# themeshpotato/rust-ray-tracing-in-a-weekend

Hardware: AMD Instinct MI355X
Metric: Msamples/s (pixels x spp) for 1200x800 random-spheres scene (higher is better)
Workload: dtype f64

## Files before the change

rust-ray-tracing-in-a-weekend_amd/csrc/abi.cpp:

```cpp
#include <hip/hip_runtime.h>

#include <algorithm>
#include <array>
#include <limits>
#include <cmath>
#include <cstdio>
#include <cstdlib>
#include <cstring>
#include <new>
#include <string>
#include <vector>

#include "rt/rt_abi.h"
#include "adaptive_criterion.hpp"
#include "ctx_internal.hpp"
#include "deal_cache.hpp"
#include "denoise.hpp"
#include "features_kernel.hpp"
#include "launch_plan.hpp"
#include "scene_lower.hpp"
#include "scene_model.hpp"
#include "trace_kernel.hpp"

namespace {
// ... 487 lines not shown
        const void* src;
        size_t bytes, off;
    } t[10] = {{L.nodes.data(), L.nodes.size() * sizeof(rt_bvh_node), 0},
               {s->prim_refs, (size_t)s->n_prim_refs * 4, 0},
               {L.prims.data(), L.prims.size() * sizeof(rt_prim), 0},
               {L.instances.data(), L.instances.size() * sizeof(rt_instance), 0},
               {s->materials, (size_t)s->n_materials * sizeof(rt_material), 0},
               {s->textures, (size_t)s->n_textures * sizeof(rt_texture), 0},
               {s->perlin_ranvec, (size_t)s->n_perlin * 768 * 8, 0},
               {s->perlin_perm, (size_t)s->n_perlin * 768 * 4, 0},
               {s->image_data, (size_t)s->image_bytes, 0},
               {L.leaf_prims.data(), L.leaf_prims.size() * sizeof(rt_prim), 0}};
    size_t total = 0;
    for (Table& e : t) {
        e.off = total;
        total = align_up(total + e.bytes, 256);
    }
    total = std::max<size_t>(total, 256);
    HIP_TRY(hipSetDevice(c->device));
    HIP_TRY(hipStreamSynchronize(c->stream));
    if (c->any_enqueued) HIP_TRY(hipEventSynchronize(c->ev_done));
    if (total > c->scene_bytes) {
        (void)hipFree(c->scene_buf);
        c->scene_buf = nullptr;
        c->scene_bytes = 0;
        HIP_TRY(hipMalloc(&c->scene_buf, total));
        c->scene_bytes = total;
    }
    char* base = (char*)c->scene_buf;
    for (const Table& e : t)
        if (e.bytes) HIP_TRY(hipMemcpy(base + e.off, e.src, e.bytes, hipMemcpyHostToDevice));

    rtk::SceneDev& S = c->S;
    S.nodes = (const rt_bvh_node*)(base + t[0].off);
    S.prim_refs = (const int32_t*)(base + t[1].off);
    S.prims = (const rt_prim*)(base + t[2].off);
    S.instances = (const rt_instance*)(base + t[3].off);
    S.materials = (const rt_material*)(base + t[4].off);
    S.textures = (const rt_texture*)(base + t[5].off);
    S.perlin_ranvec = (const double*)(base + t[6].off);
    S.perlin_perm = (const int32_t*)(base + t[7].off);
    S.image = (const uint8_t*)(base + t[8].off);
    S.leaf_prims = (const rt_prim*)(base + t[9].off);
    S.tlas_root = s->tlas_root;
    S.pre_leaf = L.pre_leaf;
    S.pre_root = L.pre_root;
    std::copy(L.pre_lo, L.pre_lo + 3, S.pre_lo);
    std::copy(L.pre_hi, L.pre_hi + 3, S.pre_hi);
    S.stack16_ok = L.stack16_ok;
    S.blas_base = L.blas_base;
    S.stack_entries = L.stack_entries;
    S.n_tlas_nodes = L.n_tlas_nodes;
    S.n_blas_bfs = L.n_blas_bfs;
    S.n_lds_nodes = S.n_lds_blas = 0;
    S.has_lights = L.has_lights;
    S.has_spheres = L.has_spheres;
    c->scene = rtp::scene_facts(L, *s);
    c->has_scene = true;
    c->stats.scene_bytes = (int64_t)total;
    return RT_OK;
}

int rt_ctx_upload_world(rt_ctx* c, rt_world* w, int accel)
{
    const rt_scene_soa* soa = nullptr;
    int rc = rt_world_flatten(w, accel, &soa);
    if (rc) return rc;
    return rt_ctx_upload_soa(c, soa);
}

int rt_rows_in_shard(int height, int row_begin, int row_stride) { return rtp::rows_in_shard(height, row_begin, row_stride); }
int rt_rows_in_band_shard(int height, int row_begin, int row_stride, int row_block)
{
    return rtp::rows_in_band_shard(height, row_begin, row_stride, row_block);
}
int rt_tiles_in_shard(int width, int height, int tile_begin, int tile_stride)
{
    return rtp::tiles_in_shard(width, height, tile_begin, tile_stride);
}
using rtp::auto_chunk;
using rtp::bad_geometry;
using rtp::Layout;
using rtp::layout_of;
using rtp::row_block_of;

static int grow(rt_ctx* c, hipStream_t stream, double*& buf, size_t& cap, size_t need, bool* oom = nullptr)
{
    if (need <= cap) return RT_OK;
    HIP_TRY(hipStreamSynchronize(stream));
    (void)hipFree(buf);
    buf = nullptr;
    cap = 0;
    const hipError_t e = hipMalloc((void**)&buf, need);
    if (e == hipErrorOutOfMemory && oom) {
        (void)hipGetLastError();
        buf = nullptr;
        *oom = true;
        return RT_ERR_HIP;
    }
    HIP_TRY(e);
    cap = need;
    return RT_OK;
}

struct Sink {
    double* acc = nullptr;
    void* out = nullptr;
// ... 139 lines not shown
static int run_range(rt_ctx* c, const rt_camera* cam, const rt_render_params* p, int s_begin, int s_end, int chunk,
                     hipStream_t stream, const Sink& sink)
{
    const Layout lay = layout_of(p);
    const long long n_px = (long long)lay.rows * lay.w;
    if (n_px == 0 || s_end <= s_begin) {
        for (int i = 0; i < 3; ++i) HIP_TRY(hipEventRecord(c->ev[i], stream));
        write_stats(c, rtp::Plan{}, chunk, 0, false);
        c->last_deal_n = 0;
        return RT_OK;
    }

    const int64_t img_tiles = (int64_t)((p->width + 7) / 8) * ((p->height + 7) / 8);
    rtk::KParams K;
    int rc = fill_kparams(c, cam, p, lay, chunk, sink, img_tiles, K);
    if (rc) return rc;

    rtp::Request rq;
    rq.lay = lay;
    rq.s_begin = s_begin;
    rq.s_end = s_end;
    rq.chunk = chunk;
    rq.count_work = p->count_work != 0;
    rq.acc_sink = sink.acc != nullptr;
    rq.moments = sink.moments != nullptr;
    rq.cam_mag = rtp::camera_magnitude(*cam);
    rtp::Retry retry{c->sample_buf_cap, true};
    rtp::Plan pl;
    for (;;) {
        pl = rtp::plan(c->scene, c->dev, c->opt, rq, retry);
        if (pl.err) return fail(pl.err, pl.err_msg);
        rc = grow(c, stream, c->acc_tmp, c->acc_tmp_cap, pl.acc_bytes);
        if (rc) return rc;
        bool oom = false;
        rc = grow(c, stream, c->partial, c->partial_cap, pl.partial_bytes, &oom);
        if (rc == RT_OK && pl.ring) {
            rc = grow(c, stream, c->ring, c->ring_cap, pl.ring_bytes, &oom);
            if (rc != RT_OK && oom) {
                retry.ring_allowed = false;
                continue;
            }
        }
        if (rc == RT_OK) break;
        if (!oom) return rc;
        if (!rtp::shrink(pl, retry)) return hip_fail(hipErrorOutOfMemory, "trace output buffer (smallest batch)");
    }
    double* const open = pl.open_chunk ? c->acc_tmp : nullptr;
    double* const acc = !pl.own_total ? sink.acc : pl.open_chunk ? c->acc_tmp + pl.px * 3 : c->acc_tmp;
    rtk::SceneDev S = c->S;
    S.n_lds_nodes = pl.n_lds_nodes;
    S.n_lds_materials = pl.n_lds_materials;
    S.n_lds_textures = pl.n_lds_textures;
    S.n_lds_blas = pl.n_lds_blas;
    K.block_chunks = pl.block_chunks;
    K.block_samples = pl.block_samples;
    K.ring_waves = pl.ring_waves;
    int waves_per_simd = 0;
    rtk::LaunchOpts o;
    o.features = pl.features;
    o.slab32 = pl.slab32;
    o.lds_stack = pl.lds_stack;
    o.count = rq.count_work;
    o.pool = pl.schedule;
    o.f32 = pl.f32;
    o.waves_per_simd = &waves_per_simd;
    const rtk::SampleTiles tiles{lay.w, lay.rows, (lay.w + 7) / 8, pl.f32};
    rc = deal_setup(c, cam, p, pl, sink.moments != nullptr, img_tiles, stream, K);
    if (rc) return rc;

    if (pl.own_total) HIP_TRY(hipMemsetAsync(acc, 0, pl.px_bytes, stream));
    if (rq.count_work) {
        HIP_TRY(hipMemsetAsync(c->counters, 0, kCounters * sizeof(unsigned long long), stream));
        if (img_tiles > c->tile_cost_cap) {
            HIP_TRY(hipStreamSynchronize(stream));
            (void)hipFree(c->tile_cost);
            c->tile_cost = nullptr;
            c->tile_cost_cap = 0;
            HIP_TRY(hipMalloc((void**)&c->tile_cost, (size_t)img_tiles * sizeof(unsigned long long)));
            c->tile_cost_cap = img_tiles;
        }
        HIP_TRY(hipMemsetAsync(c->tile_cost, 0, (size_t)img_tiles * sizeof(unsigned long long), stream));
        K.tile_cost = c->tile_cost;
        c->tile_cost_n = pl.schedule == RT_SCHED_POOL || pl.schedule == RT_SCHED_ITEMS ? img_tiles : 0;
    }
    HIP_TRY(hipEventRecord(c->ev[0], stream));
    if (pl.overlap) {
        HIP_TRY(hipEventRecord(c->ev_in, stream));
        for (int i = 0; i < 2; ++i) HIP_TRY(hipStreamWaitEvent(c->tstream[i], c->ev_in, 0));
    }
    for (int bi = 0; bi < pl.n_batches; ++bi) {
        const int b0 = s_begin + (int)(bi * pl.batch);
        const int b1 = (int)std::min<long long>(s_end, b0 + pl.batch);
        K.sample_begin = b0;
        K.spp = b1;
        K.n_chunks = (b1 - b0 + chunk - 1) / chunk;
        {
            const bool items = pl.schedule == RT_SCHED_ITEMS;
            const unsigned g = items ? (unsigned)K.block_chunks : (unsigned)K.block_samples;
            const unsigned n = items ? (unsigned)K.n_chunks : (unsigned)(K.spp - K.sample_begin);
            const unsigned n_groups = (n + g - 1) / std::max(g, 1u);
            K.n_work_blocks = (unsigned)K.tiles_x * (unsigned)K.tiles_y * n_groups;
            K.deal_div = K.tile_major ? n_groups : (unsigned)K.tiles_x * (unsigned)K.tiles_y;
        }
        const int h = pl.overlap ? (bi & 1) : 0;
        double* buf = c->partial + (size_t)h * (pl.half_bytes / sizeof(double));
        hipStream_t ts = pl.overlap ? c->tstream[h] : stream;
// ... 932 lines not shown
```

rust-ray-tracing-in-a-weekend_amd/csrc/launch_plan.cpp:

```cpp
#include "launch_plan.hpp"

#include <algorithm>
#include <cmath>

#include "launch_shapes.hpp"
#include "scene_features.hpp"

namespace rtp {

namespace {

constexpr int kMaxLdsStack = 48;
constexpr int kMaxLdsNodes = 512;
#ifndef RT_MIN_WAVES_FINAL
#define RT_MIN_WAVES_FINAL 4
#endif
#ifndef RT_LDS_BLAS_MAX
#define RT_LDS_BLAS_MAX 1024
#endif
constexpr int kMaxLdsBlas = RT_LDS_BLAS_MAX;
constexpr int kMaxLdsMaterials = 64;

}

// ... 95 lines not shown
    const size_t px_bytes = pl.px_bytes = pl.px * 3 * sizeof(double);
    const size_t sample_bytes = pl.sample_bytes =
        rtk::tiled_pixels(rq.lay.w, n_rows) * 3 * (pl.f32 ? sizeof(float) : sizeof(double));
    pl.n_lds_nodes = opt.lds_nodes ? std::min(scene.n_tlas_nodes, kMaxLdsNodes) : 0;
    const bool stage = opt.lds_nodes && scene.n_materials <= kMaxLdsMaterials && scene.n_textures <= kMaxLdsMaterials &&
                       scene.n_materials > 0;
    pl.n_lds_materials = stage ? scene.n_materials : 0;
    pl.n_lds_textures = stage ? scene.n_textures : 0;
    pl.n_lds_blas = 0;
    if (scene.n_blas_bfs > 0 && opt.lds_nodes && (variant & rtk::FEAT_INST_BLAS) != 0) {
        const bool oct = pl.slab32 && pl.n_lds_nodes == scene.n_tlas_nodes && pl.n_lds_nodes > 0;
        const int bt = rtk::block_threads_of(variant, pl.f32 != 0);
        const size_t base = (size_t)pl.n_lds_nodes * (oct ? 80 : 64) +
                            (pl.lds_stack ? (size_t)scene.stack_entries * (size_t)bt * 4 : 0) +
                            (size_t)pl.n_lds_materials * 64 + (size_t)pl.n_lds_textures * 96;
        const size_t lds_cu = dev.lds_per_cu, granule = 1024;
        const size_t wave_blocks = std::max<size_t>(1, (size_t)(variant == rtk::FEAT_SET_FINAL ? 4 * RT_MIN_WAVES_FINAL : 12) /
                                                           (size_t)(bt / 64));
        const size_t blocks = std::max<size_t>(1, std::min(wave_blocks,
            lds_cu / (((std::max<size_t>(base, 1) + granule - 1) / granule) * granule)));
        const size_t budget = std::min(lds_cu / blocks, dev.lds_per_block) / granule * granule;
        const size_t spare = budget > base ? budget - base : 0;
        pl.n_lds_blas = (int32_t)std::min<size_t>({(size_t)scene.n_blas_bfs, spare / 64, (size_t)kMaxLdsBlas});
    }
    pl.block_chunks = opt.block_chunks > 0 ? opt.block_chunks : 2;
    if (opt.block_samples > 0) {
        pl.block_samples = opt.block_samples;
    } else {
        const long long tiles = (long long)((rq.lay.w + 7) / 8) * ((n_rows + 7) / 8);
        int bs = chunk;
        while (bs > 4 && tiles * ((total + bs - 1) / bs) < 160000) bs = (bs + 1) / 2;
        pl.block_samples = bs;
    }
    const bool ring_ok = retry.ring_allowed && opt.ring && pl.block_samples == chunk &&
                         chunk <= (int)(rtk::kRingSlot / 64) && rq.s_end <= (int)rtk::kRingSampleMask;
    const int ring_waves = dev.n_cus * (variant == rtk::FEAT_SET_SPHERES ? 24 : 20);
    const size_t ring_bytes = (size_t)ring_waves * rtk::kRingWaveDoubles * sizeof(double);
    const size_t buf_cap = retry.buf_cap;

    const bool cornell = variant == rtk::FEAT_SET_RECTINST;
    const bool fits_one = (size_t)total * sample_bytes <= buf_cap;
    pl.schedule = rq.moments                     ? RT_SCHED_POOL
                  : opt.schedule != RT_SCHED_AUTO ? opt.schedule
                  : cornell && !pl.f32 ? RT_SCHED_ITEMS
                  : (ring_ok || (size_t)total * sample_bytes <= 4 * buf_cap ? RT_SCHED_POOL : RT_SCHED_ITEMS);
    pl.ring = pl.schedule == RT_SCHED_POOL && ring_ok && (opt.ring == 2 || !fits_one) && !rq.moments;
    size_t out_cap = buf_cap;
    if (pl.ring) {
        const size_t all = (size_t)pl.n_chunks * px_bytes;
        const int rings = opt.overlap && all + ring_bytes > buf_cap ? 2 : 1;
        out_cap = std::max(buf_cap > rings * ring_bytes ? buf_cap - rings * ring_bytes : 0, px_bytes);
    }
    pl.per_sample = pl.schedule == RT_SCHED_POOL && !pl.ring;
    const size_t unit = pl.per_sample ? sample_bytes : px_bytes;
    long long fit = (long long)std::max<size_t>(1, out_cap / unit);
    pl.batch = std::min<long long>(total, pl.per_sample ? fit : fit * chunk);
    const bool big_wg = rtk::block_threads_of(variant, pl.f32 != 0,
                                              rtk::stack16_launch(pl.slab32, pl.lds_stack, pl.n_lds_nodes,
                                                                  scene.n_tlas_nodes, scene.stack16_ok != 0)) > 256;
    pl.overlap = opt.overlap && !big_wg && pl.batch < total && pl.schedule != RT_SCHED_CHUNKS;
    if (pl.overlap) {
        fit = (long long)std::max<size_t>(1, out_cap / 2 / unit);
        pl.batch = std::min<long long>(total, pl.per_sample ? fit : fit * chunk);
    }
    pl.n_batches = (int)((total + pl.batch - 1) / pl.batch);
    if (pl.per_sample && !rq.moments && (pl.n_batches > 1 || rq.acc_sink)) {
        pl.open_chunk = true;
        pl.own_total = !rq.acc_sink;
        pl.acc_bytes = 2 * px_bytes;
    } else if (!pl.per_sample && pl.n_batches > 1 && !rq.acc_sink) {
        pl.own_total = true;
        pl.acc_bytes = px_bytes;
    }
    const int max_chunks = (int)((pl.batch + chunk - 1) / chunk);
    pl.half_bytes = pl.per_sample ? (size_t)pl.batch * sample_bytes : (size_t)max_chunks * px_bytes;
    pl.partial_bytes = pl.overlap ? 2 * pl.half_bytes : pl.half_bytes;
    pl.ring_waves = pl.ring ? ring_waves : 0;
    pl.ring_one_bytes = pl.ring ? ring_bytes : 0;
    pl.ring_bytes = (pl.overlap ? 2 : 1) * pl.ring_one_bytes;
    pl.trace_buf_bytes = pl.partial_bytes + pl.ring_bytes;
    return pl;
}

bool shrink(const Plan& pl, Retry& retry)
{
    if (retry.buf_cap <= ((size_t)1 << 20) || pl.partial_bytes <= (pl.per_sample ? pl.sample_bytes : pl.px_bytes))
        return false;
    retry.buf_cap = std::max<size_t>(retry.buf_cap / 2, (size_t)1 << 20);
    return true;
}

}
```

rust-ray-tracing-in-a-weekend_amd/csrc/launch_plan.hpp:

```cpp
#pragma once

#include <cstddef>
#include <cstdint>

#include "rt/rt_abi.h"
#include "scene_lower.hpp"

namespace rtp {

int rows_in_shard(int height, int row_begin, int row_stride);
int rows_in_band_shard(int height, int row_begin, int row_stride, int row_block);
int tiles_in_shard(int width, int height, int tile_begin, int tile_stride);
int row_block_of(const rt_render_params* p);
struct Layout {
    int w, rows;
};
Layout layout_of(const rt_render_params* p);
bool bad_geometry(const rt_render_params* p);
int auto_chunk(int spp);

struct SceneFacts {
    uint32_t features = 4095;
    int n_tlas_nodes = 0;
    int n_nodes = 0;
    int n_blas_bfs = 0, stack_entries = 0, stack16_ok = 0;
    int n_materials = 0, n_textures = 0;
    double pad_extent = 0.0;
};
SceneFacts scene_facts(const rtl::Lowered& L, const rt_scene_soa& s);

struct DeviceFacts {
    int n_cus = 256;
    size_t lds_per_cu = 160 * 1024;
    size_t lds_per_block = 160 * 1024;
};

struct Options {
    int slab32 = 1, lds_stack = 1, lds_nodes = 1;
    int schedule = RT_SCHED_AUTO;
    int precision = RT_PREC_F64;
    int ring = 1;
    int overlap = 1;
    int block_chunks = 0;
    int block_samples = 0;
    uint32_t extra_features = 0;
};

struct Request {
    Layout lay{0, 0};
    int s_begin = 0, s_end = 0, chunk = 1;
    bool count_work = false;
    bool acc_sink = false;
    bool moments = false;
    double cam_mag = 0.0;
};
double camera_magnitude(const rt_camera& cam);

struct Retry {
    size_t buf_cap = 0;
    bool ring_allowed = true;
};

struct Plan {
    int err = RT_OK;
    const char* err_msg = "";
    uint32_t features = 0;
    uint32_t variant = 0;
    int slab32 = 0, lds_stack = 0, f32 = 0;
    int schedule = 0;
    int n_lds_nodes = 0, n_lds_materials = 0, n_lds_textures = 0, n_lds_blas = 0;
    int block_chunks = 0, block_samples = 0;
    bool ring = false;
    int ring_waves = 0;
    bool per_sample = false;
    long long total = 0;
    int n_chunks = 0;
    long long batch = 0;
    int n_batches = 0;
    bool overlap = false;
    size_t px = 1;
    size_t px_bytes = 0;
    size_t sample_bytes = 0;
    size_t half_bytes = 0;
    size_t partial_bytes = 0;
    size_t ring_one_bytes = 0;
    size_t ring_bytes = 0;
    size_t trace_buf_bytes = 0;
    bool open_chunk = false, own_total = false;
    size_t acc_bytes = 0;
};

Plan plan(const SceneFacts& scene, const DeviceFacts& dev, const Options& opt, const Request& rq, const Retry& retry);

bool shrink(const Plan& pl, Retry& retry);

}
```

rust-ray-tracing-in-a-weekend_amd/csrc/launch_shapes.hpp:

```cpp
#pragma once

#include <cstddef>
#include <cstdint>

#ifdef __HIPCC__
#include <hip/hip_runtime.h>
#define RT_LS_HD __host__ __device__
#else
#define RT_LS_HD
#endif

#ifndef RT_BLOCK_FINAL
#define RT_BLOCK_FINAL 1024
#endif

namespace rtk {

#ifndef RT_BLOCK_F32_FINAL
#define RT_BLOCK_F32_FINAL RT_BLOCK_FINAL
#endif
#ifndef RT_BLOCK_SPHERES
#define RT_BLOCK_SPHERES 768
#endif
#ifndef RT_BLOCK_F32_SPHERES
#define RT_BLOCK_F32_SPHERES 512
#endif

#ifndef RT_STACK16
#define RT_STACK16 1
#endif
RT_LS_HD constexpr int block_threads_of(uint32_t variant_features, bool f32, bool s16 = false)
{
    return variant_features == 287u             ? (f32 ? RT_BLOCK_F32_FINAL : RT_BLOCK_FINAL)
           : variant_features == 0u  && s16 ? (f32 ? RT_BLOCK_F32_SPHERES : RT_BLOCK_SPHERES)
                                                                   : 256;
}
RT_LS_HD constexpr bool stack16_launch(bool slab32, bool lds_stack, int n_lds_nodes, int n_tlas_nodes, bool stack16_ok)
{
    return RT_STACK16 && slab32 && lds_stack && n_lds_nodes > 0 && n_lds_nodes == n_tlas_nodes && stack16_ok;
}

constexpr int kPoolRing = 4;
constexpr unsigned kRingSlot = 16 * 64;
constexpr int kRingCur = kPoolRing;
constexpr int kRingOcc = kPoolRing + 1;
constexpr size_t kRingWaveDoubles = (size_t)kPoolRing * kRingSlot * 3 + 8;
constexpr int kRingSampleBits = 20;
constexpr uint32_t kRingSampleMask = (1u << kRingSampleBits) - 1;
static_assert(kPoolRing * kRingSlot <= (1u << (32 - kRingSampleBits)), "ring record index bits");

RT_LS_HD inline size_t tiled_pixels(int width, int n_rows)
{
    return (size_t)((width + 7) / 8) * (size_t)((n_rows + 7) / 8) * 64;
}

}
```

rust-ray-tracing-in-a-weekend_amd/csrc/trace_device.hpp:

```cpp
#pragma once
#include <hip/hip_runtime.h>

#include <algorithm>
#include <type_traits>

#include "rt/rt_numerics.h"
#include "rt/rt_scene.h"
#include "trace_kernel.hpp"

namespace rtk {

typedef float f2v __attribute__((ext_vector_type(2)));
template <class R>
struct RayT {
    R ox, oy, oz;
    R dx, dy, dz;
    R time;
    R a;
    R ya;
    R ix, iy, iz;
    R yx, yy, yz;
    f2v sx, sy, sz;
    uint32_t onx, ony, onz;
};
// ... 17 lines not shown
struct Keyed {
    uint64_t seed;
    uint32_t pixel, sample, bounce;
};

struct Count {
    uint32_t casts, nodes, prims;
    uint32_t wave_steps, wave_nodes;
    uint32_t wave_leaves;
    uint32_t cam_lanes, cam_steps;
    uint32_t shade_lanes, shade_steps;
    uint64_t t_nodes, t_leaves;
    uint64_t t_setup, t_pre, t_rec, t_med, t_inst, t_refill, t_defer;
    uint64_t t_seed, t_tries;
    uint32_t idle_tail, idle_ring, no_scatter, depth_cap, try_wait;
};
#define RT_STAMP(acc, tp)                                                   \
    do {                                                                    \
        if (C::COUNT) {                                                     \
            const uint64_t t_ = __builtin_amdgcn_s_memtime();               \
            if (first_active_lane()) (acc) += t_ - (tp);                    \
            (tp) = t_;                                                      \
        }                                                                   \
    } while (0)
__device__ __forceinline__ bool first_active_lane()
{
    return (int)(threadIdx.x & 63) == __ffsll((long long)__ballot(1)) - 1;
}

#ifndef RT_RECT_RCP
#define RT_RECT_RCP 1
#endif
#ifndef RT_BOX_RCP
#define RT_BOX_RCP 1
#endif
#ifndef RT_TRY_LEFT
#define RT_TRY_LEFT 4
#endif
#ifndef RT_TRY_MIN
#define RT_TRY_MIN 2
#endif
template <class C>
constexpr bool TryLeft() { return RT_TRY_LEFT > 0 && (C::F == FEAT_SET_SPHERES || C::F == FEAT_SET_RECTINST); }
template <uint32_t F_, bool S32_, bool LDS_, bool NALL_, bool COUNT_, bool F32_ = false>
struct Cfg {
    static constexpr uint32_t F = F_;
    static constexpr bool S32 = S32_;
    static constexpr bool LDS = LDS_;
    static constexpr bool NALL = NALL_;
    static constexpr bool COUNT = COUNT_;
    static constexpr bool F32 = F32_;
    static constexpr int BT = block_threads_of(F_, F32_, RT_STACK16 && LDS_ && NALL_ && S32_);
    using Real = typename std::conditional<F32_, float, double>::type;
};

template <class C>
constexpr int BlockThreads() { return C::BT; }

template <class C, uint32_t DROP>
struct CfgDrop : C {
    static constexpr uint32_t F = C::F & ~DROP;
};
template <class C, uint32_t DROP>
struct CfgDropStatic : C {
    static constexpr uint32_t F = (C::F & ~DROP) | ((C::F & FEAT_NEST_MOVING) ? 0u : (uint32_t)FEAT_STATIC);
};
template <class C>
using InstC = CfgDropStatic<C, (C::F & FEAT_INST_RECT) ? 0u : (uint32_t)FEAT_RECT>;
template <class C>
using BoundC = CfgDropStatic<C, FEAT_INST_MEDIUM | ((C::F & FEAT_MEDIUM_INST) ? 0u : (uint32_t)(FEAT_RECT | FEAT_INST))>;
template <class C>
using InstMedC = CfgDropStatic<C, FEAT_INST_MEDIUM>;

extern __shared__ int rt_lds[];
__device__ __forceinline__ int lane_remat()
{
    int l;
    asm volatile("v_mbcnt_lo_u32_b32 %0, -1, 0\n\tv_mbcnt_hi_u32_b32 %0, -1, %0" : "=v"(l));
    return l;
}
template <bool LDS, bool REMAT = false, int BT = 256>
struct Stack;
template <int BT>
struct Stack<true, true, BT> {
    int wave0;
    __device__ __forceinline__ int& operator[](int i) const { return rt_lds[wave0 + lane_remat() + i * BT]; }
    __device__ __forceinline__ void init(int stack_off)
    {
        wave0 = stack_off + __builtin_amdgcn_readfirstlane((int)threadIdx.x & ~63);
    }
};
template <int BT>
struct Stack<true, false, BT> {
    int* base;
    __device__ __forceinline__ int& operator[](int i) const { return base[i * BT]; }
    __device__ __forceinline__ void init(int stack_off) { base = rt_lds + stack_off + threadIdx.x; }
};
template <int BT>
struct Stack<false, false, BT> {
    int v[66];
    __device__ __forceinline__ int& operator[](int i) { return v[i]; }
};
#ifndef RT_STACK16
#define RT_STACK16 1
#endif
template <int BT>
// ... 466 lines not shown
    n.child[0] = (int)d.x;
    n.child[1] = (int)d.y;
    return n;
}

__device__ __forceinline__ Node load_node_lds(uint32_t addr);

struct LdsNode {
    float ax[3][6];
    int32_t child[2];
};
static_assert(sizeof(LdsNode) == 80, "LdsNode layout");
template <class C>
constexpr bool OctNodes() { return C::NALL && C::S32; }
__device__ __forceinline__ uint32_t lds_addr(const void* p) { return (uint32_t)(uintptr_t)p; }
template <class T>
__device__ __forceinline__ const __attribute__((address_space(3))) T* lds_ptr(uint32_t a)
{
    return (const __attribute__((address_space(3))) T*)(uintptr_t)a;
}
template <class C>
constexpr int lds_node_bytes()
{
    return OctNodes<C>() ? (int)sizeof(LdsNode) : (int)sizeof(rt_bvh_node);
}
__device__ __forceinline__ Node load_node_lds(uint32_t addr)
{
    typedef unsigned u4v __attribute__((ext_vector_type(4)));
    const auto q = lds_ptr<u4v>(addr);
    const u4v a = q[0], b = q[1], c = q[2], d = q[3];
    Node n;
    n.lo0[0] = __uint_as_float(a.x); n.lo0[1] = __uint_as_float(a.y); n.lo0[2] = __uint_as_float(a.z);
    n.hi0[0] = __uint_as_float(a.w); n.hi0[1] = __uint_as_float(b.x); n.hi0[2] = __uint_as_float(b.y);
    n.lo1[0] = __uint_as_float(b.z); n.lo1[1] = __uint_as_float(b.w); n.lo1[2] = __uint_as_float(c.x);
    n.hi1[0] = __uint_as_float(c.y); n.hi1[1] = __uint_as_float(c.z); n.hi1[2] = __uint_as_float(c.w);
    n.child[0] = (int)d.x;
    n.child[1] = (int)d.y;
    return n;
}

template <class C>
constexpr bool StageShade() { return C::F != FEAT_SET_SPHERES; }
struct LdsLayout {
    size_t blas, stack, shade, total;
};
__host__ __device__ constexpr LdsLayout lds_layout(int n_nodes, int node_bytes, int n_blas, int stack_entries,
                                                   int entry_bytes, int n_materials, int n_textures, int lanes)
{
    const size_t blas = (size_t)n_nodes * (size_t)node_bytes;
    const size_t stack = blas + (size_t)n_blas * sizeof(rt_bvh_node);
    const size_t shade = stack + (size_t)stack_entries * (size_t)lanes * (size_t)entry_bytes;
    return LdsLayout{blas, stack, shade, shade + (size_t)n_materials * 64 + (size_t)n_textures * 96};
}
#ifndef RT_STAGE_BLAS
#define RT_STAGE_BLAS 1
#endif
template <class C>
constexpr bool StageBlas() { return RT_STAGE_BLAS && (C::F & FEAT_INST_BLAS) != 0; }
template <class C>
__device__ __forceinline__ LdsLayout lds_layout_of(const SceneDev& S)
{
    return lds_layout(S.n_lds_nodes, lds_node_bytes<C>(), StageBlas<C>() ? S.n_lds_blas : 0, C::LDS ? S.stack_entries : 0,
                      Stack16Cfg<C>() ? 2 : 4, StageShade<C>() ? S.n_lds_materials : 0,
                      StageShade<C>() ? S.n_lds_textures : 0, BlockThreads<C>());
}

template <class C, bool NL = false, class LeafFn, class R = typename C::Real>
__device__ __forceinline__ bool traverse(const SceneDev& S, int root, const RayT<R>& r, R t_min, R t_max,
                                         HitRefT<R>& best, StackT<C>& stack, int sp0, Count& cnt, LeafFn&& leaf)
{
    const rt_bvh_node* lds_nodes =
        reinterpret_cast<const rt_bvh_node*>(rt_lds);
    bool any = false;
    constexpr int DONE = Stack16Cfg<C>() ? -32768 : RT_DONE;
    constexpr int SSTR = C::LDS ? BlockThreads<C>() : 1;
    auto* sptr = &stack[sp0];
    using SE = typename std::remove_reference<decltype(*sptr)>::type;
    *sptr = (SE)DONE;
    sptr += SSTR;
    auto push = [&](int v) { *sptr = (SE)v; sptr += SSTR; };
    auto pop = [&]() -> int { sptr -= SSTR; return (int)*sptr; };
    int cur = root;
    float tmin_f = 0.0f, tmax_f = 0.0f;
    if constexpr (C::S32) {
        tmin_f = f32_down(t_min);
        tmax_f = f32_up(t_max);
    }
    constexpr bool OCT = NL && OctNodes<C>();
    float ninf = -__builtin_inff();
    if constexpr (OCT) asm("s_mov_b32 %0, 0xff800000" : "=s"(ninf));
    const char* const lb = reinterpret_cast<const char*>(lds_nodes);
    uint32_t blas_lds_base = 0;
    if constexpr (!NL && StageBlas<C>()) blas_lds_base = lds_addr(lb) + (uint32_t)lds_layout_of<C>(S).blas;
    (void)blas_lds_base;
    if constexpr (OCT) cur = cur >= 0 ? (int)(lds_addr(lb) + (uint32_t)cur * (uint32_t)sizeof(LdsNode)) : cur;
    auto visit = [&](int node) -> int {
        if (C::COUNT) cnt.nodes++;
        if constexpr (OCT) {
            const uint32_t nb = (uint32_t)node;
            typedef float f2v __attribute__((ext_vector_type(2)));
            typedef int i2v __attribute__((ext_vector_type(2)));
            auto pairs = [&](uint32_t off, f2v& n, f2v& f) {
                const auto q = lds_ptr<f2v>(nb + off);
                n = q[0];
                f = q[1];
            };
// ... 1016 lines not shown
            atomicAdd(&counters[5], (unsigned long long)t_shade);
            atomicAdd(&counters[8], (unsigned long long)cnt.t_nodes);
            atomicAdd(&counters[9], (unsigned long long)cnt.t_leaves);
        }
    }
}

template <class R>
__device__ __forceinline__ void forget(HitT<R>& h)
{
    h.t = __builtin_nondeterministic_value(h.t);
    h.px = __builtin_nondeterministic_value(h.px);
    h.py = __builtin_nondeterministic_value(h.py);
    h.pz = __builtin_nondeterministic_value(h.pz);
    h.nx = __builtin_nondeterministic_value(h.nx);
    h.ny = __builtin_nondeterministic_value(h.ny);
    h.nz = __builtin_nondeterministic_value(h.nz);
    h.uv0 = __builtin_nondeterministic_value(h.uv0);
    h.uv1 = __builtin_nondeterministic_value(h.uv1);
    h.uv2 = __builtin_nondeterministic_value(h.uv2);
    h.uv3 = __builtin_nondeterministic_value(h.uv3);
    h.front = __builtin_nondeterministic_value(h.front);
    h.mat = __builtin_nondeterministic_value(h.mat);
    h.uvkind = __builtin_nondeterministic_value(h.uvkind);
}

__device__ __forceinline__ unsigned lanes_below(uint64_t mask)
{
    return __builtin_amdgcn_mbcnt_hi((uint32_t)(mask >> 32), __builtin_amdgcn_mbcnt_lo((uint32_t)mask, 0u));
}

#ifndef RING_LOADS
#define RING_LOADS 4
#endif
__device__ __forceinline__ int ring_set(int val, int q, int v) { return (int)__lane_id() == q ? val : v; }

template <class C>
__device__ __forceinline__ double* ring_of_wave(const KParams& P)
{
    const unsigned wave = __builtin_amdgcn_readfirstlane(blockIdx.x * (unsigned)(BlockThreads<C>() / 64) + threadIdx.x / 64u);
    return P.ring + (size_t)wave * kRingWaveDoubles;
}
__device__ __forceinline__ unsigned* ring_block_id(double* ring_wave)
{
    return reinterpret_cast<unsigned*>(ring_wave + (size_t)kPoolRing * kRingSlot * 3);
}
template <class C>
constexpr bool RingSgpr() { return C::F == FEAT_SET_SPHERES; }
#ifndef RT_DEAL
#define RT_DEAL 3
#endif
template <class C>
constexpr bool DealCfg() { return RT_DEAL != 0 && deal_variant(C::F) && !C::COUNT; }

__device__ __forceinline__ void ring_reduce(const KParams& P, const double* __restrict__ rec,
                                            double* __restrict__ partial, unsigned blk, unsigned n_tiles, unsigned group,
                                            size_t n_px, int lane)
{
    const unsigned outer = blk / P.deal_div, inner = blk - outer * P.deal_div;
    const unsigned grp = P.tile_major ? inner : outer, tile = P.tile_major ? outer : inner;
    const int s0 = P.sample_begin + (int)(grp * group);
    const int x = (int)(tile % (unsigned)P.tiles_x) * 8 + (lane & 7);
    const int k = (int)(tile / (unsigned)P.tiles_x) * 8 + (lane >> 3);
    const int ns = min(P.spp, s0 + (int)group) - s0;
    __builtin_amdgcn_fence(__ATOMIC_RELEASE, "workgroup");
    __builtin_amdgcn_fence(__ATOMIC_ACQUIRE, "workgroup");
    constexpr int NB = RING_LOADS;
    const bool own = x < P.width && k < P.n_rows;
    double* o = partial + ((size_t)grp * n_px + (size_t)k * P.width + x) * 3;
#pragma unroll 1
    for (int c = 0; c < 3; ++c) {
        const double* p = rec + (size_t)lane * 3 + c;
        double a = 0.0;
#pragma unroll 1
        for (int j0 = 0; j0 < ns; j0 += NB) {
            double v[NB];
#pragma unroll
            for (int j = 0; j < NB; ++j) v[j] = j0 + j < ns ? p[(size_t)j * 64 * 3] : 0.0;
#pragma unroll
            for (int j = 0; j < NB; ++j)
                if (j0 + j < ns) a = a + v[j];
            p += (size_t)NB * 64 * 3;
        }
        if (own) o[c] = a;
    }
}

template <class C, bool ITEMS, bool RING = false>
__global__ void __launch_bounds__(BlockThreads<C>(), min_waves<C>()) trace_pool(SceneDev S, const KParams* __restrict__ Pp,
                                                                  double* __restrict__ samples,
                                                                  unsigned long long* __restrict__ counters,
                                                                  unsigned* __restrict__ work)
{
    const KParams& P = *Pp;
    stage_lds<C>(S);
    StackT<C> stack;
    if constexpr (Stack16Cfg<C>()) stack.base = reinterpret_cast<short*>(rt_lds + lds_stack_offset<C>(S)) + threadIdx.x;
    else if constexpr (C::LDS) stack.init((int)lds_stack_offset<C>(S));
    Count cnt{};
    uint64_t t_cam = 0, t_trace = 0, t_shade = 0, t_prev = 0, t_start = 0, t_sample = 0;
    if (C::COUNT) t_prev = t_start = __builtin_amdgcn_s_memtime();
    (void)t_trace;
    (void)t_start;
    (void)t_sample;
    const int lane = threadIdx.x & 63;
    const unsigned n_tiles = (unsigned)P.tiles_x * (unsigned)P.tiles_y;
// ... 80 lines not shown
                    if (__builtin_expect(P.tile_major != 0, 0)) {
                        tile = b / P.deal_div;
                        grp = b - tile * P.deal_div;
                        if constexpr (DealCfg<C>()) {
                            if (P.tile_major >= kDealOrdered) {
                                tile = work[kDealTable + tile];
                                if (ring) b = tile * P.deal_div + grp;
                                if ((RT_DEAL & 2) && P.tile_major == kDealMeasure) {
                                    const unsigned prev = (unsigned)(tk0 >> 3) * (unsigned)P.tiles_x + (unsigned)(tx0 >> 3);
                                    if ((blk_units == 0 || prev != tile) && lane == 0) {
                                        const unsigned now = (unsigned)__builtin_amdgcn_s_memtime();
                                        if (blk_units != 0) atomicAdd(&work[kDealTable + n_tiles + prev], now);
                                        atomicAdd(&work[kDealTable + n_tiles + tile], 0u - now);
                                    }
                                }
                            }
                        }
                    } else {
                        grp = b / n_tiles;
                        tile = b - grp * n_tiles;
                    }
                } else {
                    const unsigned outer = b / P.deal_div, inner = b - outer * P.deal_div;
                    grp = P.tile_major ? inner : outer;
                    tile = P.tile_major ? outer : inner;
                }
                tx0 = (int)(tile % (unsigned)P.tiles_x) * 8;
                tk0 = (int)(tile / (unsigned)P.tiles_x) * 8;
                vw = min(8, P.width - tx0);
                nvalid = (unsigned)(vw * min(8, P.n_rows - tk0));
                if constexpr (ITEMS) {
                    const unsigned chunk = grp * group;
                    s0 = P.sample_begin + (int)chunk * P.spp_chunk;
                    blk_units = nvalid * min(group, (unsigned)P.n_chunks - chunk);
                } else {
                    s0 = P.sample_begin + (int)(grp * group);
                    blk_units = nvalid * (unsigned)(min(P.spp, s0 + (int)group) - s0);
                    if (ring) {
                        if constexpr (RingSgpr<C>()) {
                            if (lane == 0) ring_block_id(ring_of_wave<C>(P))[free_slot] = b;
                            cur_slot = (unsigned)free_slot;
                            occ |= 1u << free_slot;
                        }
                        if constexpr (!RingSgpr<C>()) {
                            ringv = ring_set((int)b, free_slot, ringv);
                            ringv = ring_set(free_slot, kRingCur, ringv);
                            ringv = ring_set((int)(occ | 1u << free_slot), kRingOcc, ringv);
                        }
                    }
                }
                blk_next = 0;
            }
            const unsigned rank = lanes_below(need);
            const unsigned take = min((unsigned)__popcll(need), blk_units - blk_next);
            if (!active && rank < take) {
                const unsigned u = blk_next + rank;
                unsigned si;
                if (nvalid == 64u) {
                    si = u >> 6;
                    x = tx0 + (int)(u & 7u);
                    k = tk0 + (int)((u >> 3) & 7u);
                } else {
                    si = u / nvalid;
                    const unsigned p = u - si * nvalid;
                    x = tx0 + (int)(p % (unsigned)vw);
                    k = tk0 + (int)(p / (unsigned)vw);
                }
                if constexpr (ITEMS) {
                    s = s0 + (int)si * P.spp_chunk;
                    left = min(P.spp, s + P.spp_chunk) - s - 1;
                    cr = cg = cb = 0.0;
                } else {
                    s = s0 + (int)si;
                    if (ring) {
                        if constexpr (!RingSgpr<C>()) cur_slot = (unsigned)__builtin_amdgcn_readlane(ringv, kRingCur);
                        s |= (int)((cur_slot * kRingSlot + si * 64u + (unsigned)((k & 7) * 8 + (x & 7))) << kRingSampleBits);
                    }
                }
                active = true;
                new_sample = true;
            }
            blk_next += take;
            need = __ballot(!active);
        }
        if (!__any(active)) break;
        if (C::COUNT && first_active_lane()) cnt.wave_steps++;
        if (C::COUNT) {
            const uint64_t idle = __ballot(!active);
            if (first_active_lane()) {
                if (exhausted) cnt.idle_tail += (uint32_t)__popcll(idle);
                else cnt.idle_ring += (uint32_t)__popcll(idle);
            }
        }
        if (!active) continue;
        if (C::COUNT) {
            unsigned long long tw = t_prev;
            for (int off = 32; off > 0; off >>= 1) {
                const unsigned long long o = __shfl_xor(tw, off);
                tw = tw > o ? tw : o;
            }
            t_prev = tw;
            RT_STAMP(cnt.t_refill, t_prev);
        }
        bool go = true;
        bool gen_wait = false;
        {
            R u = 0, v = 0;
            bool tries = false;
            if (new_sample) {
                if (TryLeft<C>() && cam_wait) {
                    u = r.dx;
                    v = r.dy;
                    cam_wait = false;
                } else {
                    if (C::COUNT) {
                        cnt.cam_lanes++;
                        if (first_active_lane()) cnt.cam_steps++;
                    }
                    int ix, y;
                    image_xy(P, x, k, ix, y);
                    if (C::COUNT) t_sample = __builtin_amdgcn_s_memtime();
                    key.pixel = (uint32_t)y * (uint32_t)P.img_width + (uint32_t)ix;
                    const uint32_t sample = ring ? (uint32_t)s & kRingSampleMask : (uint32_t)s;
                    key.sample = sample;
                    if constexpr (C::F32) ds_start_f32(st, P.seed, key.pixel, sample);
                    else ds_start(st, P.seed, key.pixel, sample);
                    camera_begin(P, ix, y, st, u, v);
                    Tr = Tg = Tb = (R)1;
                    if constexpr (!ITEMS) cr = cg = cb = 0.0;
                    depth = P.max_depth;
                }
                tries = true;
            } else if (pending) {
                tries = shade_draws<C>(S, h.mat);
            }
            RT_STAMP(cnt.t_seed, t_prev);
            R qx = (R)0, qy = (R)0, qz = (R)0, l2 = (R)1;
            const bool three = !new_sample;
            if constexpr (TryLeft<C>()) {
                bool accepted = !tries;
                for (int n = 1;; ++n) {
                    if (!accepted) accepted = unit_try(st, (R)P.scale_m11, three, qx, qy, qz, l2);
                    const uint64_t rejecting = __ballot(!accepted);
                    if (rejecting == 0 || (n >= RT_TRY_MIN && __popcll(rejecting) <= RT_TRY_LEFT)) break;
                }
                gen_wait = !accepted;
            } else {
                while (tries && !unit_try(st, (R)P.scale_m11, three, qx, qy, qz, l2)) {
                }
            }
            RT_STAMP(cnt.t_tries, t_prev);
            if (gen_wait) {
                go = false;
                if (new_sample) {
                    cam_wait = true;
                    r.dx = u;
                    r.dy = v;
                }
            } else if (new_sample) {
                new_sample = false;
                camera_end(P, st, u, v, qx, qy, r);
            } else if (pending) {
                pending = false;
// ... 101 lines not shown
        atomicAdd(&counters[30], (unsigned long long)cnt.depth_cap);
        atomicAdd(&counters[31], (unsigned long long)cnt.try_wait);
        if (lane == 0) {
            const unsigned long long life = __builtin_amdgcn_s_memtime() - t_start;
            atomicAdd(&counters[21], life);
            atomicMax(&counters[25], life);
            atomicAdd(&counters[26], 1ull);
        }
    }
}

struct Launch {
    const SceneDev* S;
    const KParams* P;
    double* out;
    unsigned long long* counters;
    unsigned* work;
    int pool;
    unsigned long long n_blocks;
    int* waves_per_simd;
    unsigned max_waves = 0;
};

template <class K>
static int blocks_per_cu(const Launch& L, K kernel, size_t lds, int bt)
{
    int per_cu = 0;
    if (hipOccupancyMaxActiveBlocksPerMultiprocessor(&per_cu, kernel, bt, lds) != hipSuccess || per_cu <= 0) per_cu = 1;
    if (L.waves_per_simd) *L.waves_per_simd = per_cu * (bt / 256);
    return per_cu;
}

template <class K>
static unsigned resident_blocks(const Launch& L, K kernel, size_t lds, int bt)
{
    static int cus = 0;
    if (!cus) {
        int dev = 0;
        (void)hipGetDevice(&dev);
        if (hipDeviceGetAttribute(&cus, hipDeviceAttributeMultiprocessorCount, dev) != hipSuccess || cus <= 0) cus = 256;
    }
    return (unsigned)(cus * blocks_per_cu(L, kernel, lds, bt));
}

template <uint32_t F, bool S32, bool LDS, bool COUNT, bool F32>
static void launch_one(const Launch& L, hipStream_t stream, bool nall)
{
    const SceneDev& S = *L.S;
    const bool s16 = RT_STACK16 && LDS && nall && S32 && F == FEAT_SET_SPHERES;
    const int node_bytes = nall && S32 ? (int)sizeof(LdsNode) : (int)sizeof(rt_bvh_node);
    const bool stage = F != FEAT_SET_SPHERES;
    const bool blas = RT_STAGE_BLAS && (F & FEAT_INST_BLAS) != 0;
    const int bt = block_threads_of(F, F32, RT_STACK16 && LDS && nall && S32), wpb = bt / 64;
    const size_t lds = lds_layout(S.n_lds_nodes, node_bytes, blas ? S.n_lds_blas : 0, LDS ? S.stack_entries : 0,
                                  s16 ? 2 : 4, stage ? S.n_lds_materials : 0, stage ? S.n_lds_textures : 0, bt).total;
    if (L.pool) {
        auto go = [&](auto kernel) {
            unsigned nb = std::min<unsigned long long>(resident_blocks(L, kernel, lds, bt), (L.n_blocks + wpb - 1) / wpb);
            if (L.max_waves) nb = std::max(1u, std::min(nb, L.max_waves / (unsigned)wpb));
            hipLaunchKernelGGL(kernel, dim3(nb), dim3(bt), lds, stream, S, L.P, L.out, L.counters, L.work);
        };
        if (L.pool == 2) {
            if (nall) go(trace_pool<Cfg<F, S32, LDS, true, COUNT, F32>, true>);
            else go(trace_pool<Cfg<F, S32, LDS, false, COUNT, F32>, true>);
        } else if (L.max_waves) {
            if (nall) go(trace_pool<Cfg<F, S32, LDS, true, COUNT, F32>, false, true>);
            else go(trace_pool<Cfg<F, S32, LDS, false, COUNT, F32>, false, true>);
        } else {
            if (nall) go(trace_pool<Cfg<F, S32, LDS, true, COUNT, F32>, false>);
            else go(trace_pool<Cfg<F, S32, LDS, false, COUNT, F32>, false>);
        }
        return;
    }
    const unsigned nb = (unsigned)((L.n_blocks + wpb - 1) / wpb);
    auto go = [&](auto kernel) {
        if (L.waves_per_simd) (void)blocks_per_cu(L, kernel, lds, bt);
        hipLaunchKernelGGL(kernel, dim3(nb), dim3(bt), lds, stream, S, L.P, L.out, L.counters);
    };
    if (nall) go(trace_chunks<Cfg<F, S32, LDS, true, COUNT, F32>>);
    else go(trace_chunks<Cfg<F, S32, LDS, false, COUNT, F32>>);
}

template <uint32_t F, bool COUNT>
static void launch_f(const Launch& L, int slab32, int lds, hipStream_t stream)
{
    const SceneDev& S = *L.S;
    bool nall = S.n_lds_nodes > 0 && S.n_lds_nodes == S.n_tlas_nodes;
    constexpr bool S16F = F == FEAT_SET_SPHERES;
    if (RT_STACK16 && S16F && slab32 && lds && !S.stack16_ok) nall = false;
    if (RT_STACK16 && S16F && slab32 && lds && nall) {
        static int static_lds = -1;
        if (static_lds < 0) {
            static_lds = 0;
            hipFuncAttributes a;
            const void* ks[4] = {(const void*)trace_pool<Cfg<F, true, true, true, COUNT, false>, false>,
                                 (const void*)trace_pool<Cfg<F, true, true, true, COUNT, false>, true>,
                                 (const void*)trace_pool<Cfg<F, true, true, true, COUNT, false>, false, true>,
                                 (const void*)trace_chunks<Cfg<F, true, true, true, COUNT, false>>};
            for (const void* k : ks)
                if (hipFuncGetAttributes(&a, k) != hipSuccess || a.sharedSizeBytes != 0) static_lds = 1;
        }
        if (static_lds) nall = false;
    }
    if (slab32) {
        if (lds) launch_one<F, true, true, COUNT, false>(L, stream, nall);
        else launch_one<F, true, false, COUNT, false>(L, stream, nall);
    } else {
        if (lds) launch_one<F, false, true, COUNT, false>(L, stream, nall);
        else launch_one<F, false, false, COUNT, false>(L, stream, nall);
    }
}

template <uint32_t F, bool COUNT>
hipError_t launch_variant(const Launch& L, const LaunchOpts& o, hipStream_t stream)
{
    launch_f<F, COUNT>(L, o.slab32, o.lds_stack, stream);
    return hipGetLastError();
}

inline bool f32_nall(const SceneDev& S, uint32_t F, bool lds)
{
    const bool nall = S.n_lds_nodes > 0 && S.n_lds_nodes == S.n_tlas_nodes;
    return nall && !(RT_STACK16 && F == FEAT_SET_SPHERES && lds && !S.stack16_ok);
}
template <uint32_t F>
hipError_t launch_variant_f32(const Launch& L, const LaunchOpts& o, hipStream_t stream)
{
    const bool nall = f32_nall(*L.S, F, o.lds_stack);
    if (o.lds_stack) launch_one<F, true, true, false, true>(L, stream, nall);
    else launch_one<F, true, false, false, true>(L, stream, nall);
    return hipGetLastError();
}

template <uint32_t F>
hipError_t launch_variant_f32_count(const Launch& L, const LaunchOpts& o, hipStream_t stream)
{
    const bool nall = f32_nall(*L.S, F, o.lds_stack);
    if (o.lds_stack) launch_one<F, true, true, true, true>(L, stream, nall);
    else launch_one<F, true, false, true, true>(L, stream, nall);
    return hipGetLastError();
}
#define RT_VARIANT_DECL(F, COUNT) \
    extern template hipError_t launch_variant<F, COUNT>(const Launch&, const LaunchOpts&, hipStream_t);
#define RT_VARIANT_F32_DECL(F) \
    extern template hipError_t launch_variant_f32<F>(const Launch&, const LaunchOpts&, hipStream_t);
RT_VARIANT_DECL(FEAT_SET_SPHERES, false)
RT_VARIANT_DECL(FEAT_SET_SPHERES, true)
RT_VARIANT_DECL(FEAT_SET_RECTINST, false)
RT_VARIANT_DECL(FEAT_SET_RECTINST, true)
RT_VARIANT_DECL(FEAT_SET_MEDIA, false)
RT_VARIANT_DECL(FEAT_SET_MEDIA, true)
RT_VARIANT_DECL(FEAT_SET_FINAL, false)
RT_VARIANT_DECL(FEAT_SET_FINAL, true)
// ... 14 lines not shown
```

rust-ray-tracing-in-a-weekend_amd/csrc/trace_kernel.hpp:

```cpp
#pragma once

#include <hip/hip_runtime.h>

#include "rt/rt_scene.h"
#include "scene_features.hpp"
#include "launch_shapes.hpp"

namespace rtk {

struct SceneDev {
    const rt_prim* prims;
    const int32_t* prim_refs;
    const rt_prim* leaf_prims;
    const rt_bvh_node* nodes;
    const rt_instance* instances;
    const rt_material* materials;
    const rt_texture* textures;
    const double* perlin_ranvec;
    const int32_t* perlin_perm;
    const uint8_t* image;
    int32_t tlas_root;
    int32_t blas_base;
    int32_t stack_entries;
    int32_t n_lds_nodes;
    int32_t n_tlas_nodes;
    int32_t has_spheres;
    int32_t has_lights;
    int32_t n_lds_materials;
    int32_t n_lds_textures;
    int32_t pre_leaf, pre_root;
    float pre_lo[3], pre_hi[3];
    int32_t stack16_ok;
    int32_t n_blas_bfs, n_lds_blas;
    int32_t pad0;
};

struct KParams {
    rt_camera cam;
    double bg[3];
    double scale_m11;
    double scale_time;
    double wm1, hm1;
    double inv_wm1, inv_hm1;
    uint64_t seed;
    int32_t width, height, spp, max_depth;
    int32_t spp_chunk, n_chunks;
    int32_t row_begin, row_stride, n_rows;
    int32_t row_block_shift;
    int32_t tiles_x, tiles_y;
    int32_t sample_begin;
    int32_t block_chunks;
    int32_t block_samples;
    uint32_t n_work_blocks;
    int32_t img_width;
    int32_t tile_shard;
    int32_t img_tiles_x;
    uint32_t tile_div_magic;
    int32_t ring_waves;
    double* ring;
    const uint32_t* tile_order;
    int32_t tile_major;
    uint32_t deal_div;
    unsigned long long* tile_cost;
};

constexpr int32_t kDealOrdered = 2, kDealMeasure = 3;
constexpr unsigned kDealTable = 16;
constexpr bool deal_variant(uint32_t variant) { return variant == FEAT_SET_SPHERES; }

struct LaunchOpts {
    uint32_t features;
    int slab32;
    int lds_stack;
    int count;
    int pool;
    int f32;
    int* waves_per_simd = nullptr;
};

struct SampleTiles {
    int32_t width, n_rows, tiles_x;
    int32_t f32_records;
};
__host__ __device__ inline size_t tiled_record(int tiles_x, int n_samples, int x, int k, int s)
{
    const size_t tile = (size_t)(k >> 3) * (size_t)tiles_x + (size_t)(x >> 3);
    return (tile * (size_t)n_samples + (size_t)s) * 64 + (size_t)(((k & 7) << 3) | (x & 7));
// ... 36 lines not shown
```

Measured before the change: 6801.

## Stage per-pixel sample seeds and camera starts in LDS for pooled sphere kernel

Adds a staged variant of the pooled f64 spheres kernel. When a wave starts a new sample row, every lane computes one pixel's RNG stream start and camera jitter together and writes them to an LDS slot. Lanes that later refill read their start from LDS, so divergent per-lane camera setup is replaced by one uniform step. The planner turns this on only when the extra LDS does not reduce resident blocks. The cost is more LDS use, a wave barrier on each row start, and more kernel instantiations.

```diff
diff --git a/rust-ray-tracing-in-a-weekend_amd/csrc/abi.cpp b/rust-ray-tracing-in-a-weekend_amd/csrc/abi.cpp
--- a/rust-ray-tracing-in-a-weekend_amd/csrc/abi.cpp
+++ b/rust-ray-tracing-in-a-weekend_amd/csrc/abi.cpp
@@ -563,7 +563,7 @@
     S.stack_entries = L.stack_entries;
     S.n_tlas_nodes = L.n_tlas_nodes;
     S.n_blas_bfs = L.n_blas_bfs;
-    S.n_lds_nodes = S.n_lds_blas = 0;
+    S.n_lds_nodes = S.n_lds_blas = S.seed_stage_bytes = 0;
     S.has_lights = L.has_lights;
     S.has_spheres = L.has_spheres;
     c->scene = rtp::scene_facts(L, *s);
@@ -809,6 +809,7 @@
     S.n_lds_materials = pl.n_lds_materials;
     S.n_lds_textures = pl.n_lds_textures;
     S.n_lds_blas = pl.n_lds_blas;
+    S.seed_stage_bytes = (int32_t)pl.seed_stage_bytes;
     K.block_chunks = pl.block_chunks;
     K.block_samples = pl.block_samples;
     K.ring_waves = pl.ring_waves;
diff --git a/rust-ray-tracing-in-a-weekend_amd/csrc/launch_plan.cpp b/rust-ray-tracing-in-a-weekend_amd/csrc/launch_plan.cpp
--- a/rust-ray-tracing-in-a-weekend_amd/csrc/launch_plan.cpp
+++ b/rust-ray-tracing-in-a-weekend_amd/csrc/launch_plan.cpp
@@ -171,6 +171,18 @@
         out_cap = std::max(buf_cap > rings * ring_bytes ? buf_cap - rings * ring_bytes : 0, px_bytes);
     }
     pl.per_sample = pl.schedule == RT_SCHED_POOL && !pl.ring;
+    const bool s16 = variant == rtk::FEAT_SET_SPHERES &&
+                     rtk::stack16_launch(pl.slab32, pl.lds_stack, pl.n_lds_nodes, scene.n_tlas_nodes, scene.stack16_ok != 0);
+    if (RT_STAGE_SEEDS && s16 && !pl.f32 && pl.schedule == RT_SCHED_POOL) {
+        const int bt = rtk::block_threads_of(variant, false, true);
+        const size_t granule = 1024, stage = rtk::seed_stage_bytes_of(bt);
+        const size_t base = ((size_t)pl.n_lds_nodes * 80 + (size_t)scene.stack_entries * (size_t)bt * 2 + 31) / 32 * 32;
+        auto resident = [&](size_t bytes) {
+            const size_t alloc = (std::max<size_t>(bytes, 1) + granule - 1) / granule * granule;
+            return alloc > dev.lds_per_block ? (size_t)0 : std::min<size_t>(std::max(1, 24 / (bt / 64)), dev.lds_per_cu / alloc);
+        };
+        if (resident(base + stage) > 0 && resident(base + stage) == resident(base)) pl.seed_stage_bytes = stage;
+    }
     const size_t unit = pl.per_sample ? sample_bytes : px_bytes;
     long long fit = (long long)std::max<size_t>(1, out_cap / unit);
     pl.batch = std::min<long long>(total, pl.per_sample ? fit : fit * chunk);
diff --git a/rust-ray-tracing-in-a-weekend_amd/csrc/launch_plan.hpp b/rust-ray-tracing-in-a-weekend_amd/csrc/launch_plan.hpp
--- a/rust-ray-tracing-in-a-weekend_amd/csrc/launch_plan.hpp
+++ b/rust-ray-tracing-in-a-weekend_amd/csrc/launch_plan.hpp
@@ -69,6 +69,7 @@
     int slab32 = 0, lds_stack = 0, f32 = 0;
     int schedule = 0;
     int n_lds_nodes = 0, n_lds_materials = 0, n_lds_textures = 0, n_lds_blas = 0;
+    size_t seed_stage_bytes = 0;
     int block_chunks = 0, block_samples = 0;
     bool ring = false;
     int ring_waves = 0;
diff --git a/rust-ray-tracing-in-a-weekend_amd/csrc/launch_shapes.hpp b/rust-ray-tracing-in-a-weekend_amd/csrc/launch_shapes.hpp
--- a/rust-ray-tracing-in-a-weekend_amd/csrc/launch_shapes.hpp
+++ b/rust-ray-tracing-in-a-weekend_amd/csrc/launch_shapes.hpp
@@ -49,6 +49,12 @@
 constexpr uint32_t kRingSampleMask = (1u << kRingSampleBits) - 1;
 static_assert(kPoolRing * kRingSlot <= (1u << (32 - kRingSampleBits)), "ring record index bits");
 
+#ifndef RT_STAGE_SEEDS
+#define RT_STAGE_SEEDS 1
+#endif
+constexpr size_t kSeedSlotBytes = 32;
+RT_LS_HD constexpr size_t seed_stage_bytes_of(int block_threads) { return kSeedSlotBytes * (size_t)block_threads; }
+
 RT_LS_HD inline size_t tiled_pixels(int width, int n_rows)
 {
     return (size_t)((width + 7) / 8) * (size_t)((n_rows + 7) / 8) * 64;
diff --git a/rust-ray-tracing-in-a-weekend_amd/csrc/trace_device.hpp b/rust-ray-tracing-in-a-weekend_amd/csrc/trace_device.hpp
--- a/rust-ray-tracing-in-a-weekend_amd/csrc/trace_device.hpp
+++ b/rust-ray-tracing-in-a-weekend_amd/csrc/trace_device.hpp
@@ -93,6 +93,11 @@
     static constexpr bool F32 = F32_;
     static constexpr int BT = block_threads_of(F_, F32_, RT_STACK16 && LDS_ && NALL_ && S32_);
     using Real = typename std::conditional<F32_, float, double>::type;
+    static constexpr bool STAGE = false;
+};
+template <class C>
+struct CfgStage : C {
+    static constexpr bool STAGE = true;
 };
 
 template <class C>
@@ -665,6 +670,7 @@
     const size_t shade = stack + (size_t)stack_entries * (size_t)lanes * (size_t)entry_bytes;
     return LdsLayout{blas, stack, shade, shade + (size_t)n_materials * 64 + (size_t)n_textures * 96};
 }
+__host__ __device__ constexpr size_t lds_seeds_offset(size_t layout_total) { return (layout_total + 31) / 32 * 32; }
 #ifndef RT_STAGE_BLAS
 #define RT_STAGE_BLAS 1
 #endif
@@ -1787,6 +1793,23 @@
 #endif
 template <class C>
 constexpr bool DealCfg() { return RT_DEAL != 0 && deal_variant(C::F) && !C::COUNT; }
+
+struct alignas(32) SeedSlot {
+    rt_pstream st;
+    double u, v;
+};
+static_assert(sizeof(SeedSlot) == kSeedSlotBytes, "a staged sample start is one slot");
+template <class C, bool ITEMS>
+constexpr bool StagedPool()
+{
+    static_assert(!C::STAGE || (Stack16Cfg<C>() && RingSgpr<C>() && !C::F32), "staged sample starts: the f64 spheres variant's 16-bit-stack kernels");
+    return C::STAGE && !ITEMS;
+}
+template <class C>
+__device__ __forceinline__ SeedSlot* seed_slots(const SceneDev& S)
+{
+    return reinterpret_cast<SeedSlot*>(reinterpret_cast<char*>(rt_lds) + lds_seeds_offset(lds_layout_of<C>(S).total));
+}
 
 __device__ __forceinline__ void ring_reduce(const KParams& P, const double* __restrict__ rec,
                                             double* __restrict__ partial, unsigned blk, unsigned n_tiles, unsigned group,
@@ -1973,6 +1996,74 @@
                 blk_next = 0;
             }
             const unsigned rank = lanes_below(need);
+            if constexpr (StagedPool<C, ITEMS>()) {
+                unsigned row, col;
+                if (nvalid == 64u) {
+                    row = blk_next >> 6;
+                    col = blk_next & 63u;
+                } else {
+                    row = blk_next / nvalid;
+                    col = blk_next - row * nvalid;
+                }
+                if (col == 0) {
+                    uint64_t t_stage = 0;
+                    if (C::COUNT) t_stage = __builtin_amdgcn_s_memtime();
+                    if ((unsigned)lane < nvalid) {
+                        int px, pk;
+                        if (nvalid == 64u) {
+                            px = tx0 + (lane & 7);
+                            pk = tk0 + (lane >> 3);
+                        } else {
+                            px = tx0 + (int)((unsigned)lane % (unsigned)vw);
+                            pk = tk0 + (int)((unsigned)lane / (unsigned)vw);
+                        }
+                        int ix, y;
+                        image_xy(P, px, pk, ix, y);
+                        SeedSlot sl;
+                        ds_start(sl.st, P.seed, (uint32_t)y * (uint32_t)P.img_width + (uint32_t)ix, (uint32_t)(s0 + (int)row));
+                        camera_begin(P, ix, y, sl.st, sl.u, sl.v);
+                        seed_slots<C>(S)[threadIdx.x] = sl;
+                    }
+                    __builtin_amdgcn_fence(__ATOMIC_RELEASE, "wavefront");
+                    __builtin_amdgcn_wave_barrier();
+                    __builtin_amdgcn_fence(__ATOMIC_ACQUIRE, "wavefront");
+                    if (C::COUNT && lane == 0) {
+                        const uint64_t dt = __builtin_amdgcn_s_memtime() - t_stage;
+                        cnt.t_seed += dt;
+                        cnt.t_refill -= dt;
+                        cnt.cam_steps++;
+                    }
+                }
+                const unsigned take = min(min((unsigned)__popcll(need), nvalid - col), blk_units - blk_next);
+                if (!active && rank < take) {
+                    const unsigned p = col + rank;
+                    if (nvalid == 64u) {
+                        x = tx0 + (int)(p & 7u);
+                        k = tk0 + (int)(p >> 3);
+                    } else {
+                        x = tx0 + (int)(p % (unsigned)vw);
+                        k = tk0 + (int)(p / (unsigned)vw);
+                    }
+                    s = s0 + (int)row;
+                    if (ring) s |= (int)((cur_slot * kRingSlot + row * 64u + (unsigned)((k & 7) * 8 + (x & 7))) << kRingSampleBits);
+                    const SeedSlot sl = seed_slots<C>(S)[(threadIdx.x & ~63u) + p];
+                    st = sl.st;
+                    r.dx = sl.u;
+                    r.dy = sl.v;
+                    Tr = Tg = Tb = (R)1;
+                    cr = cg = cb = 0.0;
+                    depth = P.max_depth;
+                    if (C::COUNT) {
+                        cnt.cam_lanes++;
+                        t_sample = __builtin_amdgcn_s_memtime();
+                    }
+                    active = true;
+                    new_sample = true;
+                }
+                blk_next += take;
+                need = __ballot(!active);
+                continue;
+            }
             const unsigned take = min((unsigned)__popcll(need), blk_units - blk_next);
             if (!active && rank < take) {
                 const unsigned u = blk_next + rank;
@@ -2029,7 +2120,10 @@
             R u = 0, v = 0;
             bool tries = false;
             if (new_sample) {
-                if (TryLeft<C>() && cam_wait) {
+                if constexpr (StagedPool<C, ITEMS>()) {
+                    u = r.dx;
+                    v = r.dy;
+                } else if (TryLeft<C>() && cam_wait) {
                     u = r.dx;
                     v = r.dy;
                     cam_wait = false;
@@ -2237,14 +2331,25 @@
     const bool stage = F != FEAT_SET_SPHERES;
     const bool blas = RT_STAGE_BLAS && (F & FEAT_INST_BLAS) != 0;
     const int bt = block_threads_of(F, F32, RT_STACK16 && LDS && nall && S32), wpb = bt / 64;
-    const size_t lds = lds_layout(S.n_lds_nodes, node_bytes, blas ? S.n_lds_blas : 0, LDS ? S.stack_entries : 0,
-                                  s16 ? 2 : 4, stage ? S.n_lds_materials : 0, stage ? S.n_lds_textures : 0, bt).total;
+    constexpr bool can_stage = RT_STAGE_SEEDS && RT_STACK16 && F == FEAT_SET_SPHERES && S32 && LDS && !F32;
+    const int seed_bytes = can_stage && nall && L.pool == 1 && S.seed_stage_bytes == (int)seed_stage_bytes_of(bt)
+                               ? S.seed_stage_bytes : 0;
+    const size_t lds_rest = lds_layout(S.n_lds_nodes, node_bytes, blas ? S.n_lds_blas : 0, LDS ? S.stack_entries : 0,
+                                       s16 ? 2 : 4, stage ? S.n_lds_materials : 0, stage ? S.n_lds_textures : 0, bt).total;
+    const size_t lds = seed_bytes ? lds_seeds_offset(lds_rest) + (size_t)seed_bytes : lds_rest;
     if (L.pool) {
         auto go = [&](auto kernel) {
             unsigned nb = std::min<unsigned long long>(resident_blocks(L, kernel, lds, bt), (L.n_blocks + wpb - 1) / wpb);
             if (L.max_waves) nb = std::max(1u, std::min(nb, L.max_waves / (unsigned)wpb));
             hipLaunchKernelGGL(kernel, dim3(nb), dim3(bt), lds, stream, S, L.P, L.out, L.counters, L.work);
         };
+        if constexpr (can_stage) {
+            if (seed_bytes) {
+                if (L.max_waves) go(trace_pool<CfgStage<Cfg<F, S32, LDS, true, COUNT, F32>>, false, true>);
+                else go(trace_pool<CfgStage<Cfg<F, S32, LDS, true, COUNT, F32>>, false>);
+                return;
+            }
+        }
         if (L.pool == 2) {
             if (nall) go(trace_pool<Cfg<F, S32, LDS, true, COUNT, F32>, true>);
             else go(trace_pool<Cfg<F, S32, LDS, false, COUNT, F32>, true>);
@@ -2284,6 +2389,12 @@
                                  (const void*)trace_chunks<Cfg<F, true, true, true, COUNT, false>>};
             for (const void* k : ks)
                 if (hipFuncGetAttributes(&a, k) != hipSuccess || a.sharedSizeBytes != 0) static_lds = 1;
+            if constexpr (RT_STAGE_SEEDS != 0 && RT_STACK16 != 0 && S16F) {
+                const void* kst[2] = {(const void*)trace_pool<CfgStage<Cfg<F, true, true, true, COUNT, false>>, false>,
+                                      (const void*)trace_pool<CfgStage<Cfg<F, true, true, true, COUNT, false>>, false, true>};
+                for (const void* k : kst)
+                    if (hipFuncGetAttributes(&a, k) != hipSuccess || a.sharedSizeBytes != 0) static_lds = 1;
+            }
         }
         if (static_lds) nall = false;
     }
diff --git a/rust-ray-tracing-in-a-weekend_amd/csrc/trace_kernel.hpp b/rust-ray-tracing-in-a-weekend_amd/csrc/trace_kernel.hpp
--- a/rust-ray-tracing-in-a-weekend_amd/csrc/trace_kernel.hpp
+++ b/rust-ray-tracing-in-a-weekend_amd/csrc/trace_kernel.hpp
@@ -32,7 +32,7 @@
     float pre_lo[3], pre_hi[3];
     int32_t stack16_ok;
     int32_t n_blas_bfs, n_lds_blas;
-    int32_t pad0;
+    int32_t seed_stage_bytes;
 };
 
 struct KParams {
```

New measurement: 7028, median of 6. +3.3%, better.
